# actionml/universal-recommender

Hardware: NVIDIA H100
Metric: CCO train events/sec to indicator model (higher is better)
Workload: dtype int32+f64

## Files before the change

### universal_recommender_b200/csrc/cco_api.cu

```cuda
#include <cuda_runtime.h>
#include <dlfcn.h>
#include <stdarg.h>
#include <stdio.h>
#include <stdlib.h>
#include <string.h>

#include <algorithm>
#include <cmath>
#include <functional>
#include <cub/cub.cuh>
#include <nvtx3/nvToolsExt.h>
#include <condition_variable>
#include <mutex>
#include <string>
#include <thread>
#include <vector>

#include "../../include/cco_b200.h"
#include "cco_kernels.cuh"
#include "cco_sampler.cuh"
#include "cco_format.cuh"
#include "cco_strings.cuh"

namespace cco {
// ... 391 lines not shown
  m.col += m.q_base;
  m.q_base = 0;
  m.nnz = n_unique;
  CK(cudaGetLastError());
  ar.release(flag);
  ar.release(pos);
  ar.release(k0);
  ar.release(k1);
  return CCO_OK;
}

struct HeavyRows {
  int32_t *list = nullptr;
  int *n = nullptr;
};
static int list_heavy_rows(cco_ctx *c, Arena &ar, const DevRaw &raw, HeavyRows *h) {
  CKR(ar.alloc(&h->list, std::max<long long>(raw.n_rows, 1)));
  CKR(ar.alloc(&h->n, 1));
  CK(cudaMemsetAsync(h->n, 0, 4, c->stream));
  if (raw.n_rows > 0) {
    k_list_heavy_rows<<<grid_for(raw.n_rows, 256, c->sm_count), 256, 0, c->stream>>>(raw.n_rows, raw.rp, h->list, h->n);
    c->launches++;
  }
  return CCO_OK;
}
static void launch_check(cco_ctx *c, const DevRaw &raw, const HeavyRows &h, int *flags) {
  if (raw.n_rows <= 0) return;
  const long long q_lo = raw.q_base, q_hi = raw.q_base + raw.nnz;
  k_check_rows<kSG><<<grid_for(raw.n_rows * kSG, 256, c->sm_count), 256, 0, c->stream>>>(raw.n_rows, raw.n_cols, raw.rp, raw.col, q_lo, q_hi,
                                                                                       nullptr, nullptr, flags);
  k_check_rows<32><<<c->sm_count * 4, 256, 0, c->stream>>>(raw.n_rows, raw.n_cols, raw.rp, raw.col, q_lo, q_hi, h.list, h.n, flags);
  c->launches += 2;
}
struct SampleScratch {
  unsigned long long *col_thr = nullptr;
  uint8_t *keep = nullptr;
};
static int sample_scratch(cco_ctx *c, Arena &ar, const DevRaw &raw, const int32_t *raw_counts, int32_t m, SampleScratch *sc) {
  CKR(ar.alloc(&sc->col_thr, std::max<int32_t>(raw.n_cols, 1)));
  CKR(ar.alloc(&sc->keep, std::max<long long>(raw.nnz, 1)));
  if (raw.n_cols > 0) {
    k_col_thresholds<<<grid_for(raw.n_cols, 256, c->sm_count, 4), 256, 0, c->stream>>>(raw.n_cols, raw_counts, m, sc->col_thr);
    c->launches++;
  }
  return CCO_OK;
}
static void launch_count(cco_ctx *c, const DevRaw &raw, const SampleScratch &sc, int32_t m, int32_t seed, uint32_t flags, const int *bad,
                         uint32_t *kept, int32_t *new_counts) {
  if (raw.n_rows <= 0 || raw.nnz <= 0) return;
  const long long q_lo = raw.q_base, q_hi = raw.q_base + raw.nnz;
  const long long n_chunks = (raw.nnz + kSampleChunk - 1) / kSampleChunk;
  k_sample_count<<<grid_for(n_chunks * 32, 256, c->sm_count), 256, 0, c->stream>>>(raw.n_rows, raw.row_base, raw.rp, raw.col, raw.n_cols, q_lo, q_hi,
                                                                                  sc.col_thr, m, seed, flags, bad, kept, new_counts, sc.keep);
  c->launches++;
}
static int launch_write(cco_ctx *c, Arena &ar, const DevRaw &raw, const SampleScratch &sc, int32_t *dst) {
  if (raw.n_rows <= 0 || raw.nnz <= 0) return CCO_OK;
  long long *n_sel;
  CKR(ar.alloc(&n_sel, 1));
  size_t tb = 0;
  CK(cub::DeviceSelect::Flagged(nullptr, tb, raw.col + raw.q_base, sc.keep, dst, n_sel, (long long)raw.nnz, c->stream));
  void *tmp;
  CKR(ar.alloc((char **)&tmp, tb));
  CK(cub::DeviceSelect::Flagged(tmp, tb, raw.col + raw.q_base, sc.keep, dst, n_sel, (long long)raw.nnz, c->stream));
  ar.release(tmp);
  c->launches += 2;
  return CCO_OK;
}

static int downsample_device(cco_ctx *c, Arena &ar, const DevRaw &raw, const int *bad, const int32_t *raw_counts, int32_t m,
                             int32_t seed, uint32_t flags, DevMat *out) {
  out->n_rows = raw.n_rows;
  out->n_cols = raw.n_cols;
  uint32_t *kept;
  CKR(ar.alloc(&kept, raw.n_rows + 1));
  CKR(ar.alloc(&out->rp, raw.n_rows + 1));
  if (!out->marg) CKR(ar.alloc(&out->marg, std::max<int32_t>(raw.n_cols, 1)));
  CKR(ar.alloc(&out->col, std::max<long long>(raw.nnz, 1)));
  CK(cudaMemsetAsync(out->marg, 0, sizeof(int32_t) * std::max<int32_t>(raw.n_cols, 1), c->stream));
  CK(cudaMemsetAsync(kept, 0, sizeof(uint32_t) * ((size_t)raw.n_rows + 1), c->stream));
  SampleScratch sc;
  CKR(sample_scratch(c, ar, raw, raw_counts, m, &sc));
  launch_count(c, raw, sc, m, seed, flags, bad, kept, out->marg);
  CKR(exclusive_sum_u32(c, ar, kept, out->rp, raw.n_rows + 1));
  CKR(launch_write(c, ar, raw, sc, out->col));
  CK(cudaGetLastError());
  ar.release(kept);
  ar.release(sc.col_thr);
  ar.release(sc.keep);
  return CCO_OK;
}

static int nccl_check(int rc, const char *what) {
  if (rc != 0) return set_error(CCO_E_NCCL, "%s: %s", what, g_nccl.GetErrorString(rc));
  return CCO_OK;
}

static int downsample_sharded_all(cco_ctx *c, Arena &ar, const std::vector<DevRaw> &raw, const int *d_check ,
                                  const std::vector<long long> &block_cap,
                                  long long U, const int32_t *raw_counts, int32_t *marg_all, const std::vector<long long> &col_off,
                                  const cco_indicator_params_t *params, int32_t seed, uint32_t flags, std::vector<DevMat> &dm,
                                  cudaEvent_t *stage_ev ) {
  cudaStream_t s = c->stream;
  const int W = c->world, r = c->rank, n_mats = (int)raw.size();
  const long long S = (U + W - 1) / W;
  const long long row_base = raw[0].row_base;
  std::vector<uint32_t *> kept(n_mats, nullptr);
  std::vector<SampleScratch> sc(n_mats);
  for (int i = 0; i < n_mats; ++i) {
    DevMat *out = &dm[i];
    out->n_rows = U;
    out->n_cols = raw[i].n_cols;
    out->marg = marg_all + col_off[i];
    CKR(ar.alloc(&kept[i], (size_t)(W * S + 1)));
    CKR(ar.alloc(&out->rp, U + 1));
    CK(cudaMemsetAsync(kept[i], 0, sizeof(uint32_t) * (size_t)(W * S + 1), s));
    CKR(sample_scratch(c, ar, raw[i], raw_counts + col_off[i], params[i].max_interactions, &sc[i]));
    launch_count(c, raw[i], sc[i], params[i].max_interactions, seed, flags, d_check + 2 * i, kept[i], out->marg);
  }
  CK(cudaEventRecord(stage_ev[0], s));
  if (S > 0) {
    g_nccl.GroupStart();
    for (int i = 0; i < n_mats; ++i) {
      int rc = g_nccl.AllGather(kept[i] + (size_t)r * S, kept[i], (size_t)S, kNcclUint32, c->comm, s);
      if (rc != 0) { g_nccl.GroupEnd(); return nccl_check(rc, "ncclAllGather(kept counts)"); }
    }
    CKR(nccl_check(g_nccl.GroupEnd(), "ncclGroupEnd(kept counts)"));
  }
  if (col_off[n_mats] > 0)
    CKR(nccl_check(g_nccl.AllReduce(marg_all, marg_all, (size_t)col_off[n_mats], kNcclInt32, kNcclSum, c->comm, s), "ncclAllReduce(marginals)"));
  std::vector<int32_t *> gathered(n_mats, nullptr);
  std::vector<uint32_t> edge((size_t)n_mats * (W + 1), 0);
  for (int i = 0; i < n_mats; ++i) {
    CKR(exclusive_sum_u32(c, ar, kept[i], dm[i].rp, U + 1));
    ar.release(kept[i]);
    for (int q = 0; q <= W; ++q) CKR(mail_fetch(c, &edge[(size_t)i * (W + 1) + q], dm[i].rp + std::min<long long>((long long)q * S, U), 4));
  }
  CK(cudaEventRecord(stage_ev[1], s));
  CKR(mail_wait(c));
  std::vector<long long> cap(n_mats, 0);
  for (int i = 0; i < n_mats; ++i) {
    for (int q = 0; q < W; ++q) cap[i] = std::max<long long>(cap[i], (long long)edge[(size_t)i * (W + 1) + q + 1] - edge[(size_t)i * (W + 1) + q]);
    CKR(ar.alloc(&dm[i].col, std::max<long long>(edge[(size_t)i * (W + 1) + W], 1)));
    if (cap[i] == 0) continue;
    CKR(ar.alloc(&gathered[i], (size_t)(cap[i] * W)));
    CKR(launch_write(c, ar, raw[i], sc[i], gathered[i] + (size_t)r * cap[i]));
    ar.release(sc[i].col_thr);
    ar.release(sc[i].keep);
  }
  CK(cudaEventRecord(stage_ev[2], s));
  g_nccl.GroupStart();
// ... 619 lines not shown
  } guard{res};
  std::vector<IndicatorState> ist(n_mats);
  for (auto &x : ist) CKR(pooled_event(c, false, &x.packed));
  cco_stats_t &st = res->stats;
  st.n_mats = n_mats;
  st.n_users = ds->n_users;
  st.ms_h2d = ds->ms_h2d;
  const bool h2d_pending = ds->h2d_pending;
  const long long n_users = ds->n_users;
  std::vector<DevRaw> raw(n_mats);
  for (int i = 0; i < n_mats; ++i) {
    raw[i].n_rows = ds->n_local;
    raw[i].row_base = ds->row_base;
    raw[i].n_cols = (int32_t)ds->n_cols[i];
    raw[i].q_base = ds->q_lo[i];
    raw[i].nnz = ds->q_hi[i] - ds->q_lo[i];
    raw[i].nnz_cap = ds->nnz[i];
    raw[i].rp = ds->rp[i];
    raw[i].col = ds->col[i];
    st.nnz_in_total += ds->nnz[i];
  }
  CK(cudaEventRecord(c->ev[1], s));
  nvtx_push("cco:prepare");
  std::vector<cudaEvent_t> sev(8, nullptr);
  for (auto &e : sev) CKR(pooled_event(c, true, &e));
  auto mark = [&](int k) { return cudaEventRecord(sev[k], s); };
  long long total_cols = 0;
  std::vector<long long> col_off(n_mats + 1, 0);
  for (int i = 0; i < n_mats; ++i) {
    col_off[i] = total_cols;
    total_cols += raw[i].n_cols;
  }
  col_off[n_mats] = total_cols;
  constexpr int kHistCopies = 16;
  const long long copy_stride = std::max<long long>(total_cols, 1);
  int32_t *raw_counts, *marg_all;
  int *d_check;
  CKR(ar.alloc(&raw_counts, (size_t)copy_stride * kHistCopies));
  CKR(ar.alloc(&marg_all, (size_t)copy_stride));
  CKR(ar.alloc(&d_check, 2 * n_mats));
  CK(cudaMemsetAsync(raw_counts, 0, sizeof(int32_t) * (size_t)copy_stride * kHistCopies, s));
  CK(cudaMemsetAsync(marg_all, 0, sizeof(int32_t) * (size_t)copy_stride, s));
  CK(cudaMemsetAsync(d_check, 0, sizeof(int) * 2 * n_mats, s));
  for (int i = 0; i < n_mats; ++i) {
    CK(cudaStreamWaitEvent(s, ds->ready[i], 0));
    if (ds->n_local == 0) continue;
    int *verdict = ds->validated ? nullptr : d_check + 2 * i;
    if (verdict) {
      k_check_row_ptr<<<grid_for(raw[i].n_rows, 256, c->sm_count), 256, 0, s>>>(raw[i].n_rows, raw[i].rp, raw[i].q_base, raw[i].q_base + raw[i].nnz,
                                                                              verdict);
      c->launches++;
    }
    if (raw[i].nnz > 0) {
      k_col_histogram_flat<true><<<grid_for(raw[i].nnz, 256, c->sm_count), 256, 0, s>>>(raw[i].nnz, raw[i].col + raw[i].q_base, raw[i].n_cols,
                                                                                       raw_counts + col_off[i], kHistCopies, copy_stride, verdict);
      c->launches++;
    }
  }
  if (total_cols > 0) {
    k_sum_copies<<<grid_for(total_cols, 256, c->sm_count), 256, 0, s>>>(total_cols, kHistCopies, copy_stride, raw_counts);
    c->launches++;
  }
  CK(mark(0));
  if (c->world > 1) {
    if (total_cols > 0)
      CKR(nccl_check(g_nccl.AllReduce(raw_counts, raw_counts, (size_t)total_cols, kNcclInt32, kNcclSum, c->comm, s), "ncclAllReduce(raw counts)"));
    CKR(nccl_check(g_nccl.AllReduce(d_check, d_check, (size_t)(2 * n_mats), kNcclInt32, kNcclMax, c->comm, s), "ncclAllReduce(check flags)"));
  }
  CK(mark(1));
  std::vector<DevMat> dm(n_mats);
  if (c->world > 1) {
    CKR(downsample_sharded_all(c, ar, raw, d_check, ds->block_cap, n_users, raw_counts, marg_all, col_off, params, seed, flags, dm, &sev[2]));
  } else {
    for (int i = 0; i < n_mats; ++i) {
      dm[i].marg = marg_all + col_off[i];
      CKR(downsample_device(c, ar, raw[i], d_check + 2 * i, raw_counts + col_off[i], params[i].max_interactions, seed, flags, &dm[i]));
    }
    CK(mark(2));
    CK(mark(3));
    CK(mark(4));
    CK(mark(5));
  }
  const int32_t n_items_a = dm[0].n_cols;
  uint32_t *at_ptr, *cursor;
  int32_t *at_users, *d_max;
  CKR(ar.alloc(&at_ptr, n_items_a + 1));
  CKR(ar.alloc(&cursor, n_items_a + 1));
  CKR(ar.alloc(&d_max, n_mats));
  CKR(ar.alloc(&at_users, std::max<long long>(ds->nnz[0], 1)));
  CK(cudaMemsetAsync(d_max, 0, 4 * (size_t)n_mats, s));
  {
    uint32_t *marg_pad;
    CKR(ar.alloc(&marg_pad, n_items_a + 1));
    CK(cudaMemcpyAsync(marg_pad, dm[0].marg, sizeof(int32_t) * (size_t)n_items_a, cudaMemcpyDeviceToDevice, s));
    CK(cudaMemsetAsync(marg_pad + n_items_a, 0, 4, s));
    CKR(exclusive_sum_u32(c, ar, marg_pad, at_ptr, (long long)n_items_a + 1));
    ar.release(marg_pad);
  }
  CK(cudaMemcpyAsync(cursor, at_ptr, sizeof(uint32_t) * ((size_t)n_items_a + 1), cudaMemcpyDeviceToDevice, s));
  k_transpose_scatter<<<grid_for(n_users * kSG, 256, c->sm_count), 256, 0, s>>>(n_users, dm[0].rp, dm[0].col, cursor, at_users);
  c->launches++;
  for (int i = 0; i < n_mats; ++i)
    if (dm[i].n_cols > 0) {
      k_max_i32<<<grid_for(dm[i].n_cols, 256, c->sm_count, 2), 256, 0, s>>>(dm[i].n_cols, dm[i].marg, d_max + i);
      c->launches++;
    }
  std::vector<int32_t> max_marg(n_mats, 0);
  std::vector<uint32_t> h_nnz(n_mats);
  std::vector<int> h_check(2 * n_mats, 0);
  CKR(mail_fetch(c, max_marg.data(), d_max, 4 * (size_t)n_mats));
  CKR(mail_fetch(c, h_check.data(), d_check, sizeof(int) * 2 * (size_t)n_mats));
  for (int i = 0; i < n_mats; ++i) CKR(mail_fetch(c, &h_nnz[i], dm[i].rp + n_users, 4));
  CK(mark(6));
  CK(cudaEventRecord(c->ev[2], s));
  nvtx_pop();
  CKR(mail_wait(c));
  for (int i = 0; i < n_mats; ++i)
    if (h_check[2 * i]) return set_error(CCO_E_INVALID_ARG, "matrix %d: row_ptr not monotone or column index out of [0, n_cols)", i);
  for (int i = 0; i < n_mats && i < 16; ++i) st.nnz_downsampled[i] = h_nnz[i];

  std::vector<IndicatorOut> io(n_mats);
  std::vector<cudaEvent_t> ev_rows(2 * n_mats, nullptr);
  for (auto &e : ev_rows) CKR(pooled_event(c, true, &e));
  for (int i = 0; i < n_mats; ++i) {
    nvtx_push("cco:indicator");
    CKR(enqueue_indicator(c, ar, at_ptr, at_users, n_items_a, dm[0].marg, max_marg[0], max_marg[i], dm[i], n_users, i == 0, params[i],
                          flags, false, c->ev[2], ev_rows[2 * i], ev_rows[2 * i + 1], &ist[i]));
    nvtx_pop();
    if (i > 0) CKR(finish_indicator(c, &ist[i - 1], flags, i - 1, &res->mats[i - 1], &io[i - 1]));
  }
  CKR(finish_indicator(c, &ist[n_mats - 1], flags, n_mats - 1, &res->mats[n_mats - 1], &io[n_mats - 1]));
  CK(cudaEventRecord(c->copy_ev[1], c->copy_stream));
  CK(cudaStreamWaitEvent(s, c->copy_ev[1], 0));
  CK(cudaEventRecord(c->ev[3], s));
// ... 1250 lines not shown
  long long *d[4];
  double *dout;
  const int64_t *h[4] = {k11, k12, k21, k22};
  for (int j = 0; j < 4; ++j) {
    CKR(ar.alloc(&d[j], n));
    CK(cudaMemcpyAsync(d[j], h[j], sizeof(int64_t) * (size_t)n, cudaMemcpyHostToDevice, c->stream));
  }
  CKR(ar.alloc(&dout, n));
  k_debug_llr<<<(unsigned)((n + 255) / 256), 256, 0, c->stream>>>(n, d[0], d[1], d[2], d[3], flags, dout);
  CK(cudaMemcpyAsync(out, dout, sizeof(double) * (size_t)n, cudaMemcpyDeviceToHost, c->stream));
  CK(cudaStreamSynchronize(c->stream));
  CK(cudaGetLastError());
  return CCO_OK;
}

int cco_debug_downsample(cco_ctx_t *c, const cco_csr_t *m, int32_t max_interactions, int32_t seed, uint32_t flags,
                         int64_t **row_ptr, int32_t **col_idx, int32_t *raw_col_counts, int32_t *new_col_counts) {
  if (!c || !m || !row_ptr || !col_idx) return set_error(CCO_E_INVALID_ARG, "null argument");
  if (c->world != 1 || !c->members.empty()) return set_error(CCO_E_UNSUPPORTED, "debug entries need a single-GPU context");
  cco_indicator_params_t prm = {max_interactions, 1, 0, 0.0};
  CKR(validate_host(1, m, &prm));
  CK(cudaSetDevice(c->device));
  mail_reset(c);
  cco_dataset *ds = nullptr;
  CKR(dataset_upload(c, 1, m, flags, &ds));
  struct DG { cco_dataset *d; ~DG() { dataset_release(d); } } dg{ds};
  Arena ar(c->stream);
  DevRaw raw;
  raw.n_rows = ds->n_users; raw.n_cols = (int32_t)ds->n_cols[0]; raw.nnz = ds->nnz[0]; raw.nnz_cap = ds->nnz[0];
  raw.rp = ds->rp[0]; raw.col = ds->col[0];
  int32_t *counts;
  CKR(ar.alloc(&counts, std::max<int32_t>(m->n_cols, 1)));
  CK(cudaMemsetAsync(counts, 0, sizeof(int32_t) * (size_t)std::max<int32_t>(m->n_cols, 1), c->stream));
  if (raw.nnz > 0 && m->n_rows > 0)
    k_col_histogram<<<grid_for(raw.nnz, 256, c->sm_count), 256, 0, c->stream>>>(0, m->n_rows, raw.rp, raw.col, raw.n_cols, counts, 1, 0);
  DevMat dm;
  CKR(downsample_device(c, ar, raw, nullptr, counts, max_interactions, seed, flags, &dm));
  std::vector<uint32_t> rp32((size_t)m->n_rows + 1);
  CK(cudaMemcpyAsync(rp32.data(), dm.rp, sizeof(uint32_t) * rp32.size(), cudaMemcpyDeviceToHost, c->stream));
  if (raw_col_counts && m->n_cols > 0)
    CK(cudaMemcpyAsync(raw_col_counts, counts, sizeof(int32_t) * (size_t)m->n_cols, cudaMemcpyDeviceToHost, c->stream));
  if (new_col_counts && m->n_cols > 0)
    CK(cudaMemcpyAsync(new_col_counts, dm.marg, sizeof(int32_t) * (size_t)m->n_cols, cudaMemcpyDeviceToHost, c->stream));
  CK(cudaStreamSynchronize(c->stream));
  CK(cudaGetLastError());
  size_t nnz = rp32[m->n_rows];
  int64_t *rp = (int64_t *)malloc(sizeof(int64_t) * rp32.size());
  int32_t *ci = (int32_t *)malloc(sizeof(int32_t) * std::max<size_t>(nnz, 1));
  if (!rp || !ci) return set_error(CCO_E_OOM, "malloc failed");
  for (size_t i = 0; i < rp32.size(); ++i) rp[i] = rp32[i];
  if (nnz) CK(cudaMemcpy(ci, dm.col, sizeof(int32_t) * nnz, cudaMemcpyDeviceToHost));
  *row_ptr = rp;
  *col_idx = ci;
  return CCO_OK;
}

int cco_debug_cooccurrence(cco_ctx_t *c, const cco_csr_t *a, const cco_csr_t *b, int64_t **row_ptr, int32_t **col_idx,
                           int32_t **count) {
  if (!c || !a || !b || !row_ptr || !col_idx || !count) return set_error(CCO_E_INVALID_ARG, "null argument");
  if (c->world != 1 || !c->members.empty()) return set_error(CCO_E_UNSUPPORTED, "debug entries need a single-GPU context");
  cco_csr_t two[2] = {*a, *b};
  cco_indicator_params_t prm[2] = {{0x7fffffff, 1, 0, 0.0}, {0x7fffffff, 1, 0, 0.0}};
  CKR(validate_host(2, two, prm));
  CK(cudaSetDevice(c->device));
  mail_reset(c);
  cudaStream_t s = c->stream;
  cco_dataset *ds = nullptr;
  CKR(dataset_upload(c, 2, two, 0, &ds));
  struct DG { cco_dataset *d; ~DG() { dataset_release(d); } } dg{ds};
  Arena ar(s);
  struct CopyJoin {
    cco_ctx *c;
    ~CopyJoin() { cudaStreamSynchronize(c->copy_stream); }
  } copy_join{c};
  std::vector<DevRaw> raw(2);
  for (int i = 0; i < 2; ++i) {
    raw[i].n_rows = ds->n_users; raw[i].n_cols = (int32_t)ds->n_cols[i]; raw[i].nnz = ds->nnz[i]; raw[i].nnz_cap = ds->nnz[i];
    raw[i].rp = ds->rp[i]; raw[i].col = ds->col[i];
  }
  std::vector<DevMat> dm(2);
  for (int i = 0; i < 2; ++i) {
    int32_t *counts;
    CKR(ar.alloc(&counts, std::max<int32_t>(raw[i].n_cols, 1)));
    CK(cudaMemsetAsync(counts, 0, sizeof(int32_t) * (size_t)std::max<int32_t>(raw[i].n_cols, 1), s));
    if (raw[i].nnz > 0 && raw[i].n_rows > 0)
      k_col_histogram<<<grid_for(raw[i].nnz, 256, c->sm_count), 256, 0, s>>>(0, raw[i].n_rows, raw[i].rp, raw[i].col, raw[i].n_cols, counts, 1, 0);
    CKR(downsample_device(c, ar, raw[i], nullptr, counts, 0x7fffffff, 0, 0, &dm[i]));
  }
  const int32_t n_items_a = dm[0].n_cols;
  uint32_t *at_ptr, *cursor, *marg_pad;
  int32_t *at_users, *d_max;
  CKR(ar.alloc(&at_ptr, n_items_a + 1));
  CKR(ar.alloc(&cursor, n_items_a + 1));
  CKR(ar.alloc(&marg_pad, n_items_a + 1));
  CKR(ar.alloc(&d_max, 2));
  CKR(ar.alloc(&at_users, std::max<long long>(raw[0].nnz, 1)));
  CK(cudaMemsetAsync(d_max, 0, 8, s));
  CK(cudaMemcpyAsync(marg_pad, dm[0].marg, sizeof(int32_t) * (size_t)n_items_a, cudaMemcpyDeviceToDevice, s));
  CK(cudaMemsetAsync(marg_pad + n_items_a, 0, 4, s));
  CKR(exclusive_sum_u32(c, ar, marg_pad, at_ptr, (long long)n_items_a + 1));
  CK(cudaMemcpyAsync(cursor, at_ptr, sizeof(uint32_t) * ((size_t)n_items_a + 1), cudaMemcpyDeviceToDevice, s));
  k_transpose_scatter<<<grid_for(a->n_rows * kSG, 256, c->sm_count), 256, 0, s>>>(a->n_rows, dm[0].rp, dm[0].col, cursor, at_users);
  if (n_items_a > 0) k_max_i32<<<grid_for(n_items_a, 256, c->sm_count, 2), 256, 0, s>>>(n_items_a, dm[0].marg, d_max);
  if (dm[1].n_cols > 0) k_max_i32<<<grid_for(dm[1].n_cols, 256, c->sm_count, 2), 256, 0, s>>>(dm[1].n_cols, dm[1].marg, d_max + 1);
  int32_t max_marg_ab[2] = {0, 0};
  CK(cudaMemcpyAsync(max_marg_ab, d_max, 8, cudaMemcpyDeviceToHost, s));
  CK(cudaStreamSynchronize(s));
  CK(cudaGetLastError());
  ResultMat rm;
  IndicatorOut io;
  IndicatorState ist;
  struct EG { IndicatorState &x; ~EG() { if (x.packed) cudaEventDestroy(x.packed); } } eg{ist};
  cco_indicator_params_t p1 = {0x7fffffff, 1, 0, 0.0};
  auto put = [&]() {
    for (void *p : {(void *)rm.row_ptr, (void *)rm.col, (void *)rm.llr, (void *)rm.cnt})
      if (p) c->pinned_put(p);
  };
  int rc = enqueue_indicator(c, ar, at_ptr, at_users, n_items_a, dm[0].marg, max_marg_ab[0], max_marg_ab[1], dm[1], a->n_rows, false, p1,
                             0, true, nullptr, nullptr, nullptr, &ist);
  if (rc == CCO_OK) rc = finish_indicator(c, &ist, 0, 0, &rm, &io);
  cudaStreamSynchronize(c->copy_stream);
  if (rc != CCO_OK) {
    put();
    return rc;
  }
  size_t nnz = (size_t)rm.row_ptr[n_items_a];
  int64_t *rp = (int64_t *)malloc(sizeof(int64_t) * ((size_t)n_items_a + 1));
  int32_t *ci = (int32_t *)malloc(sizeof(int32_t) * std::max<size_t>(nnz, 1));
  int32_t *cn = (int32_t *)malloc(sizeof(int32_t) * std::max<size_t>(nnz, 1));
  if (!rp || !ci || !cn) {
    put();
    return set_error(CCO_E_OOM, "malloc failed");
  }
  memcpy(rp, rm.row_ptr, sizeof(int64_t) * ((size_t)n_items_a + 1));
  std::vector<std::pair<int32_t, int32_t>> tmp;
// ... 19 lines not shown
```

### universal_recommender_b200/csrc/cco_kernels.cuh

```cuda
#pragma once

#include <cuda_runtime.h>
#include <stdint.h>

namespace cco {

struct RowArgs {
  const uint32_t *at_ptr;
  const int32_t *at_users;
  const uint32_t *b_ptr;
  const int32_t *b_col;
  const int32_t *marg_a;
  const int32_t *marg_b;
  const int32_t *key_of_col;
  const int32_t *first_key_of_cb;
  int32_t key_shift;
  const uint2 *ext;
  int32_t max_marg_b;
  const int32_t *rows_sorted;
  const uint32_t *row_work;
  const int32_t *bin_bounds;
  int32_t bin;
  int32_t n_cols_b;
  long long n_users;
// ... 94 lines not shown

constexpr int kHeavyRow = 256;
__global__ void k_list_heavy_rows(long long n_rows, const long long *__restrict__ rp, int32_t *__restrict__ list, int *__restrict__ n_list) {
  for (long long r = blockIdx.x * (long long)blockDim.x + threadIdx.x; r < n_rows; r += (long long)gridDim.x * blockDim.x)
    if (rp[r + 1] - rp[r] > kHeavyRow) list[atomicAdd(n_list, 1)] = (int32_t)r;
}
#define CCO_ROW_LOOP_BEGIN(SG)                                                                         \
  const int lane = threadIdx.x % SG;                                                                   \
  long long it = (blockIdx.x * (long long)blockDim.x + threadIdx.x) / SG;                              \
  const long long stride = (long long)gridDim.x * blockDim.x / SG;                                     \
  const long long n_it = list ? (long long)*n_list : n_rows;                                           \
  for (; it < n_it; it += stride) {                                                                    \
    const long long row = list ? (long long)list[it] : it;
#define CCO_ROW_LOOP_END }

template <int SG>
__global__ void k_check_rows(long long n_rows, int32_t n_cols, const long long *__restrict__ rp, const int32_t *__restrict__ col,
                             long long q_lo, long long q_hi, const int32_t *__restrict__ list, const int *__restrict__ n_list, int *flags) {
  int bad = 0, unsorted = 0;
  CCO_ROW_LOOP_BEGIN(SG)
    long long s = rp[row], e = rp[row + 1];
    if (e < s || s < q_lo || e > q_hi) { bad = 1; continue; }
    if (!list && e - s > kHeavyRow) continue;
    for (long long q = s + lane; q < e; q += SG) {
      int32_t c = col[q];
      if (c < 0 || c >= n_cols) bad = 1;
      if (q > s && col[q - 1] >= c) unsorted = 1;
    }
  CCO_ROW_LOOP_END
  if (bad) atomicOr(&flags[0], 1);
  if (unsorted) atomicOr(&flags[1], 1);
}

__global__ void k_col_histogram(long long row_begin, long long row_end, const long long *__restrict__ rp,
                                const int32_t *__restrict__ col, int32_t n_cols, int32_t *__restrict__ counts, int n_copies,
                                long long copy_stride) {
  const long long s = rp[row_begin], e = rp[row_end];
  const int lane = threadIdx.x & 31;
  int32_t *mine = counts + (long long)(blockIdx.x % n_copies) * copy_stride;
  for (long long q0 = s + blockIdx.x * (long long)blockDim.x + (threadIdx.x & ~31); q0 < e;
       q0 += (long long)gridDim.x * blockDim.x) {
    const long long q = q0 + lane;
    const bool act = q < e;
    const unsigned am = __ballot_sync(0xffffffffu, act);
    if (act) {
      int32_t c = col[q];
      unsigned peers = __match_any_sync(am, c);
      if ((__ffs(peers) - 1) == lane && (uint32_t)c < (uint32_t)n_cols) atomicAdd(&mine[c], __popc(peers));
    }
  }
}
__global__ void k_sum_copies(long long n, int n_copies, long long copy_stride, int32_t *__restrict__ counts) {
  for (long long i = blockIdx.x * (long long)blockDim.x + threadIdx.x; i < n; i += (long long)gridDim.x * blockDim.x) {
    int32_t acc = counts[i];
    for (int k = 1; k < n_copies; ++k) acc += counts[i + k * copy_stride];
    counts[i] = acc;
  }
}

__global__ void k_col_histogram_u32(const uint32_t *__restrict__ lo, const uint32_t *__restrict__ hi,
                                    const int32_t *__restrict__ col, int32_t *__restrict__ counts) {
  const long long s = *lo, e = *hi;
  const int lane = threadIdx.x & 31;
  for (long long q0 = s + blockIdx.x * (long long)blockDim.x + (threadIdx.x & ~31); q0 < e;
       q0 += (long long)gridDim.x * blockDim.x) {
    const long long q = q0 + lane;
    const bool act = q < e;
    const unsigned am = __ballot_sync(0xffffffffu, act);
    if (act) {
      const int32_t c = col[q];
      const unsigned peers = __match_any_sync(am, c);
      if ((__ffs(peers) - 1) == lane) atomicAdd(&counts[c], __popc(peers));
    }
  }
}

__device__ __forceinline__ double row_sample_rate(long long d, int32_t m, bool intdiv) {
  if (d <= 0) return 1.0;
  const long long md = d < m ? d : (long long)m;
  return intdiv ? (double)(md / d) : __ddiv_rn((double)md, (double)d);
}
constexpr unsigned long long kKeepAlways = 1ULL << 53;
__device__ __forceinline__ unsigned long long rate_threshold(double rate) {
  if (rate >= 1.0) return kKeepAlways;
  return (unsigned long long)floor(__dmul_rn(rate, 0x1.0p53));
}
__global__ void k_col_thresholds(int32_t n_cols, const int32_t *__restrict__ raw_counts, int32_t m, unsigned long long *__restrict__ thr) {
  for (int j = blockIdx.x * blockDim.x + threadIdx.x; j < n_cols; j += gridDim.x * blockDim.x) {
    const int32_t c = raw_counts[j];
    thr[j] = c <= m ? kKeepAlways : rate_threshold(__ddiv_rn((double)m, (double)c));
  }
}
// ... 40 lines not shown
                                   long long q_lo, long long q_hi, const uint8_t *__restrict__ keep_flag,
                                   const int32_t *__restrict__ list, const int *__restrict__ n_list,
                                   const uint32_t *__restrict__ new_ptr, const uint32_t *__restrict__ out_base, int32_t *__restrict__ new_col) {
  const int sg_shift = SG == 32 ? 0 : (threadIdx.x & 31) / SG * SG;
  const unsigned sg_mask = SG == 32 ? 0xffffffffu : (((1u << SG) - 1u) << sg_shift);
  const uint32_t base = out_base ? *out_base : 0u;
  CCO_ROW_LOOP_BEGIN(SG)
    long long s = rp[row], e = rp[row + 1], d = e - s;
    if (!list && d > kHeavyRow) continue;
    if (d < 0 || s < q_lo || e > q_hi) continue;
    uint32_t w = new_ptr[row_base + row] - base;
    for (long long q0 = s; q0 < e; q0 += SG) {
      long long q = q0 + lane;
      bool keep = false;
      int32_t j = 0;
      if (q < e) {
        j = col[q];
        keep = keep_flag[q - q_lo] != 0;
      }
      unsigned b = (__ballot_sync(sg_mask, keep) & sg_mask) >> sg_shift;
      if (keep) new_col[w + __popc(b & ((1u << lane) - 1u))] = j;
      w += __popc(b);
    }
  CCO_ROW_LOOP_END
}

__global__ void k_pack_blocks(int world, long long S, long long U, long long cap, const uint32_t *__restrict__ new_ptr,
                              const int32_t *__restrict__ gathered, int32_t *__restrict__ new_col) {
  for (int q = blockIdx.y; q < world; q += gridDim.y) {
    const long long u0 = min((long long)q * S, U), u1 = min(u0 + S, U);
    const uint32_t lo = new_ptr[u0], hi = new_ptr[u1];
    const int32_t *src = gathered + (long long)q * cap;
    for (uint32_t i = blockIdx.x * blockDim.x + threadIdx.x; i < hi - lo; i += gridDim.x * blockDim.x) new_col[lo + i] = src[i];
  }
}

__global__ void k_transpose_scatter(long long n_rows, const uint32_t *__restrict__ rp, const int32_t *__restrict__ col,
                                    uint32_t *__restrict__ cursor, int32_t *__restrict__ users) {
  const int lane = threadIdx.x % kSG;
  long long row = (blockIdx.x * (long long)blockDim.x + threadIdx.x) / kSG;
  const long long stride = (long long)gridDim.x * blockDim.x / kSG;
  for (; row < n_rows; row += stride) {
    uint32_t s = rp[row], e = rp[row + 1];
    for (uint32_t q = s + lane; q < e; q += kSG) users[atomicAdd(&cursor[col[q]], 1u)] = (int32_t)row;
  }
}

__global__ void k_row_work(int32_t n_items, const uint32_t *__restrict__ at_ptr, const int32_t *__restrict__ at_users,
                           const uint32_t *__restrict__ b_ptr, uint32_t *__restrict__ row_work,
                           unsigned long long *__restrict__ work64, int32_t *__restrict__ item_ids,
                           uint2 *__restrict__ ext) {
  const int lane = threadIdx.x % kSG;
  const unsigned sg_mask = ((1u << kSG) - 1u) << ((threadIdx.x & 31) / kSG * kSG);
  int item = (blockIdx.x * blockDim.x + threadIdx.x) / kSG;
  const int stride = gridDim.x * blockDim.x / kSG;
  for (; item < n_items; item += stride) {
    uint32_t s = at_ptr[item], e = at_ptr[item + 1];
    unsigned long long w = 0;
    for (uint32_t q = s + lane; q < e; q += kSG) {
      int32_t u = at_users[q];
      const uint32_t bs = b_ptr[u], bl = b_ptr[u + 1] - bs;
      w += bl;
      if (ext) ext[q] = make_uint2(bs, bl);
    }
#pragma unroll
    for (int o = kSG / 2; o > 0; o >>= 1) w += __shfl_xor_sync(sg_mask, w, o);
    if (lane == 0) {
      row_work[item] = w > 0xffffffffULL ? 0xffffffffu : (uint32_t)w;
      work64[item] = w;
      item_ids[item] = item;
    }
  }
}

struct BinThresholds {
  uint32_t t[12];
};
// ... 782 lines not shown
```

### universal_recommender_b200/csrc/cco_sampler.cuh

```cuda
#pragma once

#include <cuda_runtime.h>
#include <stdint.h>

#include "cco_kernels.cuh"

namespace cco {

constexpr int kSampleChunk = 256;

__device__ __forceinline__ long long warp_find_row(const long long *__restrict__ rp, long long n_rows, long long q, int lane) {
  long long lo = 0, hi = n_rows;
  while (hi - lo > 1) {
    const long long step = (hi - lo + 31) / 32;
    const long long p = lo + lane * step;
    const bool ok = p < hi && rp[p] <= q;
    const unsigned b = __ballot_sync(0xffffffffu, ok) | 1u;
    const int top = 31 - __clz(b);
    lo += top * step;
    hi = hi < lo + step ? hi : lo + step;
  }
  return lo;
}

__global__ void __launch_bounds__(256) k_sample_count(long long n_rows, long long row_base, const long long *__restrict__ rp,
                                                      const int32_t *__restrict__ col, int32_t n_cols, long long q_lo, long long q_hi,
                                                      const unsigned long long *__restrict__ col_thr, int32_t m, int32_t seed, uint32_t flags,
                                                      const int *__restrict__ bad ,
                                                      uint32_t *__restrict__ kept_per_row , int32_t *__restrict__ new_counts,
                                                      uint8_t *__restrict__ keep_flag) {
  const int lane = threadIdx.x & 31;
  const long long warp = (blockIdx.x * (long long)blockDim.x + threadIdx.x) >> 5;
  const long long n_warps = ((long long)gridDim.x * blockDim.x) >> 5;
  const long long n_chunks = (q_hi - q_lo + kSampleChunk - 1) / kSampleChunk;
  const bool intdiv = (flags & CCO_FLAG_ROWRATE_INTDIV) != 0;
  const long long kNoRow = 0x7fffffffffffffffLL;
  if (n_rows <= 0) return;
  if (bad && *bad) {
    for (long long q = blockIdx.x * (long long)blockDim.x + threadIdx.x; q < q_hi - q_lo; q += (long long)gridDim.x * blockDim.x) keep_flag[q] = 0;
    return;
  }
  for (long long chunk = warp; chunk < n_chunks; chunk += n_warps) {
    const long long Q0 = q_lo + chunk * kSampleChunk;
    const long long Q1 = Q0 + kSampleChunk < q_hi ? Q0 + kSampleChunk : q_hi;
    long long base = warp_find_row(rp, n_rows, Q0, lane);
    long long start_i, end_i;
    unsigned long long t_i, x_i;
    uint32_t kept_i;
#define CCO_LOAD_WINDOW()                                                                                   \
  {                                                                                                         \
    const long long r = base + lane;                                                                        \
    start_i = end_i = kNoRow;                                                                               \
    t_i = kKeepAlways;                                                                                      \
    x_i = 0;                                                                                                \
    if (r < n_rows) {                                                                                       \
      start_i = rp[r];                                                                                      \
      end_i = rp[r + 1];                                                                                    \
      const long long d = end_i - start_i;                                                                  \
      if (d > (long long)m) t_i = rate_threshold(row_sample_rate(d, m, intdiv));  \
      x_i = mix64(((uint64_t)(uint32_t)seed << 32) | (uint64_t)(uint32_t)(row_base + r));                   \
    }                                                                                                       \
    kept_i = 0;                                                                                             \
  }
#define CCO_FLUSH_WINDOW()                                                                                  \
  if (kept_i) atomicAdd(&kept_per_row[row_base + base + lane], kept_i);
    CCO_LOAD_WINDOW()
    for (long long qb = Q0; qb < Q1; qb += 32) {
      const long long q = qb + lane;
      bool pending = q < Q1;
      const int32_t j = pending ? col[q] : 0;
      unsigned long long t_col = kKeepAlways;
      if (pending && (uint32_t)j < (uint32_t)n_cols) t_col = col_thr[j];
      while (true) {
        int idx = 0;
#pragma unroll
        for (int step = 16; step > 0; step >>= 1) {
          const long long v = __shfl_sync(0xffffffffu, end_i, idx + step - 1);
          if (v <= q) idx += step;
        }
        {
          const long long v = __shfl_sync(0xffffffffu, end_i, idx);
          if (v <= q) idx += 1;
        }
        const int src = idx & 31;
        const unsigned long long t_row = __shfl_sync(0xffffffffu, t_i, src);
        const unsigned long long x_row = __shfl_sync(0xffffffffu, x_i, src);
        const bool here = pending && idx < 32;
        const bool real_row = base + idx < n_rows;
        bool keep = false;
        if (here) {
          keep = real_row && (uint32_t)j < (uint32_t)n_cols && keep_entry_thr(t_row, t_col, x_row, (uint32_t)j);
          keep_flag[q - q_lo] = keep ? 1 : 0;
          if (keep && new_counts) atomicAdd(&new_counts[j], 1);
        }
        const unsigned kb = __ballot_sync(0xffffffffu, keep);
        const int a = start_i <= qb ? 0 : (start_i >= qb + 32 ? 32 : (int)(start_i - qb));
        const int b = end_i <= qb ? 0 : (end_i >= qb + 32 ? 32 : (int)(end_i - qb));
        if (b > a) {
          const unsigned below_b = b >= 32 ? 0xffffffffu : ((1u << b) - 1u);
          const unsigned below_a = (1u << a) - 1u;
          kept_i += __popc(kb & below_b & ~below_a);
        }
        pending = pending && !here;
        if (!__any_sync(0xffffffffu, pending)) break;
        CCO_FLUSH_WINDOW()
        base += 32;
        if (base >= n_rows) {
          if (pending) keep_flag[q - q_lo] = 0;
          kept_i = 0;
          start_i = end_i = kNoRow;
          break;
        }
        CCO_LOAD_WINDOW()
      }
      if (base >= n_rows) {
        for (long long q2 = qb + 32 + lane; q2 < Q1; q2 += 32) keep_flag[q2 - q_lo] = 0;
        break;
      }
    }
    if (base < n_rows && base + lane < n_rows) { CCO_FLUSH_WINDOW() }
#undef CCO_LOAD_WINDOW
#undef CCO_FLUSH_WINDOW
  }
}

__global__ void k_check_row_ptr(long long n_rows, const long long *__restrict__ rp, long long q_lo, long long q_hi, int *flags) {
  int bad = 0;
  for (long long r = blockIdx.x * (long long)blockDim.x + threadIdx.x; r < n_rows; r += (long long)gridDim.x * blockDim.x) {
    const long long s = rp[r], e = rp[r + 1];
    if (e < s || s < q_lo || e > q_hi) bad = 1;
  }
  if (bad) atomicOr(&flags[0], 1);
}
template <bool AGG>
__global__ void k_col_histogram_flat(long long n, const int32_t *__restrict__ col, int32_t n_cols, int32_t *__restrict__ counts, int n_copies,
                                     long long copy_stride, int *flags ) {
  int32_t *mine = counts + (long long)(blockIdx.x % n_copies) * copy_stride;
  const int lane = threadIdx.x & 31;
  int bad = 0;
  for (long long q0 = blockIdx.x * (long long)blockDim.x + (threadIdx.x & ~31); q0 < n; q0 += (long long)gridDim.x * blockDim.x) {
    const long long q = q0 + lane;
    const bool act = q < n;
    const int32_t j = act ? col[q] : -1;
    const bool ok = act && (uint32_t)j < (uint32_t)n_cols;
    if (act && !ok) bad = 1;
    if (AGG) {
      const unsigned om = __ballot_sync(0xffffffffu, ok);
      if (ok) {
        const unsigned peers = __match_any_sync(om, j);
        if ((__ffs(peers) - 1) == lane) atomicAdd(&mine[j], __popc(peers));
      }
    } else if (ok) {
      atomicAdd(&mine[j], 1);
    }
  }
  if (flags && bad) atomicOr(&flags[0], 1);
}

}
```

Baseline: 4.037 billion.

## Rework column histogram, sampler partitioning, and transpose into entry-balanced kernels

```diff
diff --git a/universal_recommender_b200/csrc/cco_api.cu b/universal_recommender_b200/csrc/cco_api.cu
--- a/universal_recommender_b200/csrc/cco_api.cu
+++ b/universal_recommender_b200/csrc/cco_api.cu
@@ -447,6 +447,22 @@
   k_check_rows<32><<<c->sm_count * 4, 256, 0, c->stream>>>(raw.n_rows, raw.n_cols, raw.rp, raw.col, q_lo, q_hi, h.list, h.n, flags);
   c->launches += 2;
 }
+static int launch_col_histogram(cco_ctx *c, const DevRaw &raw, int32_t *counts, int *verdict, cudaStream_t s) {
+  if (raw.nnz <= 0) return CCO_OK;
+  CK(cudaFuncSetAttribute(k_col_histogram_hot, cudaFuncAttributeMaxDynamicSharedMemorySize, (int)(2 * kHotSlots * sizeof(uint32_t))));
+  const long long grid = std::max<long long>(c->sm_count, (raw.nnz >> 30) + 1);
+  k_col_histogram_hot<<<(unsigned)grid, 1024, 2 * kHotSlots * sizeof(uint32_t), s>>>(raw.nnz, raw.col + raw.q_base, raw.n_cols, counts, verdict);
+  c->launches++;
+  return CCO_OK;
+}
+static int launch_transpose(cco_ctx *c, long long n_rows, const uint32_t *rp, const int32_t *col, uint32_t *cursor, int32_t *users,
+                            cudaStream_t s) {
+  int occ = 1;
+  CK(cudaOccupancyMaxActiveBlocksPerMultiprocessor(&occ, k_transpose_entries, 256, 0));
+  k_transpose_entries<<<c->sm_count * std::max(occ, 1), 256, 0, s>>>(n_rows, rp, col, cursor, users);
+  c->launches++;
+  return CCO_OK;
+}
 struct SampleScratch {
   unsigned long long *col_thr = nullptr;
   uint8_t *keep = nullptr;
@@ -460,14 +476,16 @@
   }
   return CCO_OK;
 }
-static void launch_count(cco_ctx *c, const DevRaw &raw, const SampleScratch &sc, int32_t m, int32_t seed, uint32_t flags, const int *bad,
-                         uint32_t *kept, int32_t *new_counts) {
-  if (raw.n_rows <= 0 || raw.nnz <= 0) return;
+static int launch_count(cco_ctx *c, const DevRaw &raw, const SampleScratch &sc, int32_t m, int32_t seed, uint32_t flags, const int *bad,
+                        uint32_t *kept, int32_t *new_counts) {
+  if (raw.n_rows <= 0 || raw.nnz <= 0) return CCO_OK;
   const long long q_lo = raw.q_base, q_hi = raw.q_base + raw.nnz;
-  const long long n_chunks = (raw.nnz + kSampleChunk - 1) / kSampleChunk;
-  k_sample_count<<<grid_for(n_chunks * 32, 256, c->sm_count), 256, 0, c->stream>>>(raw.n_rows, raw.row_base, raw.rp, raw.col, raw.n_cols, q_lo, q_hi,
+  int occ = 1;
+  CK(cudaOccupancyMaxActiveBlocksPerMultiprocessor(&occ, k_sample_count, 256, 0));
+  k_sample_count<<<grid_for((raw.nnz + 7) / 8, 256, c->sm_count, std::max(occ, 1)), 256, 0, c->stream>>>(raw.n_rows, raw.row_base, raw.rp, raw.col, raw.n_cols, q_lo, q_hi,
                                                                                   sc.col_thr, m, seed, flags, bad, kept, new_counts, sc.keep);
   c->launches++;
+  return CCO_OK;
 }
 static int launch_write(cco_ctx *c, Arena &ar, const DevRaw &raw, const SampleScratch &sc, int32_t *dst) {
   if (raw.n_rows <= 0 || raw.nnz <= 0) return CCO_OK;
@@ -496,7 +514,7 @@
   CK(cudaMemsetAsync(kept, 0, sizeof(uint32_t) * ((size_t)raw.n_rows + 1), c->stream));
   SampleScratch sc;
   CKR(sample_scratch(c, ar, raw, raw_counts, m, &sc));
-  launch_count(c, raw, sc, m, seed, flags, bad, kept, out->marg);
+  CKR(launch_count(c, raw, sc, m, seed, flags, bad, kept, out->marg));
   CKR(exclusive_sum_u32(c, ar, kept, out->rp, raw.n_rows + 1));
   CKR(launch_write(c, ar, raw, sc, out->col));
   CK(cudaGetLastError());
@@ -531,7 +549,7 @@
     CKR(ar.alloc(&out->rp, U + 1));
     CK(cudaMemsetAsync(kept[i], 0, sizeof(uint32_t) * (size_t)(W * S + 1), s));
     CKR(sample_scratch(c, ar, raw[i], raw_counts + col_off[i], params[i].max_interactions, &sc[i]));
-    launch_count(c, raw[i], sc[i], params[i].max_interactions, seed, flags, d_check + 2 * i, kept[i], out->marg);
+    CKR(launch_count(c, raw[i], sc[i], params[i].max_interactions, seed, flags, d_check + 2 * i, kept[i], out->marg));
   }
   CK(cudaEventRecord(stage_ev[0], s));
   if (S > 0) {
@@ -1217,15 +1235,14 @@
     total_cols += raw[i].n_cols;
   }
   col_off[n_mats] = total_cols;
-  constexpr int kHistCopies = 16;
-  const long long copy_stride = std::max<long long>(total_cols, 1);
+  const long long n_counts = std::max<long long>(total_cols, 1);
   int32_t *raw_counts, *marg_all;
   int *d_check;
-  CKR(ar.alloc(&raw_counts, (size_t)copy_stride * kHistCopies));
-  CKR(ar.alloc(&marg_all, (size_t)copy_stride));
+  CKR(ar.alloc(&raw_counts, (size_t)n_counts));
+  CKR(ar.alloc(&marg_all, (size_t)n_counts));
   CKR(ar.alloc(&d_check, 2 * n_mats));
-  CK(cudaMemsetAsync(raw_counts, 0, sizeof(int32_t) * (size_t)copy_stride * kHistCopies, s));
-  CK(cudaMemsetAsync(marg_all, 0, sizeof(int32_t) * (size_t)copy_stride, s));
+  CK(cudaMemsetAsync(raw_counts, 0, sizeof(int32_t) * (size_t)n_counts, s));
+  CK(cudaMemsetAsync(marg_all, 0, sizeof(int32_t) * (size_t)n_counts, s));
   CK(cudaMemsetAsync(d_check, 0, sizeof(int) * 2 * n_mats, s));
   for (int i = 0; i < n_mats; ++i) {
     CK(cudaStreamWaitEvent(s, ds->ready[i], 0));
@@ -1236,15 +1253,7 @@
                                                                               verdict);
       c->launches++;
     }
-    if (raw[i].nnz > 0) {
-      k_col_histogram_flat<true><<<grid_for(raw[i].nnz, 256, c->sm_count), 256, 0, s>>>(raw[i].nnz, raw[i].col + raw[i].q_base, raw[i].n_cols,
-                                                                                       raw_counts + col_off[i], kHistCopies, copy_stride, verdict);
-      c->launches++;
-    }
-  }
-  if (total_cols > 0) {
-    k_sum_copies<<<grid_for(total_cols, 256, c->sm_count), 256, 0, s>>>(total_cols, kHistCopies, copy_stride, raw_counts);
-    c->launches++;
+    CKR(launch_col_histogram(c, raw[i], raw_counts + col_off[i], verdict, s));
   }
   CK(mark(0));
   if (c->world > 1) {
@@ -1283,8 +1292,7 @@
     ar.release(marg_pad);
   }
   CK(cudaMemcpyAsync(cursor, at_ptr, sizeof(uint32_t) * ((size_t)n_items_a + 1), cudaMemcpyDeviceToDevice, s));
-  k_transpose_scatter<<<grid_for(n_users * kSG, 256, c->sm_count), 256, 0, s>>>(n_users, dm[0].rp, dm[0].col, cursor, at_users);
-  c->launches++;
+  CKR(launch_transpose(c, n_users, dm[0].rp, dm[0].col, cursor, at_users, s));
   for (int i = 0; i < n_mats; ++i)
     if (dm[i].n_cols > 0) {
       k_max_i32<<<grid_for(dm[i].n_cols, 256, c->sm_count, 2), 256, 0, s>>>(dm[i].n_cols, dm[i].marg, d_max + i);
@@ -2601,8 +2609,7 @@
   int32_t *counts;
   CKR(ar.alloc(&counts, std::max<int32_t>(m->n_cols, 1)));
   CK(cudaMemsetAsync(counts, 0, sizeof(int32_t) * (size_t)std::max<int32_t>(m->n_cols, 1), c->stream));
-  if (raw.nnz > 0 && m->n_rows > 0)
-    k_col_histogram<<<grid_for(raw.nnz, 256, c->sm_count), 256, 0, c->stream>>>(0, m->n_rows, raw.rp, raw.col, raw.n_cols, counts, 1, 0);
+  if (m->n_rows > 0) CKR(launch_col_histogram(c, raw, counts, nullptr, c->stream));
   DevMat dm;
   CKR(downsample_device(c, ar, raw, nullptr, counts, max_interactions, seed, flags, &dm));
   std::vector<uint32_t> rp32((size_t)m->n_rows + 1);
@@ -2652,8 +2659,7 @@
     int32_t *counts;
     CKR(ar.alloc(&counts, std::max<int32_t>(raw[i].n_cols, 1)));
     CK(cudaMemsetAsync(counts, 0, sizeof(int32_t) * (size_t)std::max<int32_t>(raw[i].n_cols, 1), s));
-    if (raw[i].nnz > 0 && raw[i].n_rows > 0)
-      k_col_histogram<<<grid_for(raw[i].nnz, 256, c->sm_count), 256, 0, s>>>(0, raw[i].n_rows, raw[i].rp, raw[i].col, raw[i].n_cols, counts, 1, 0);
+    if (raw[i].n_rows > 0) CKR(launch_col_histogram(c, raw[i], counts, nullptr, s));
     CKR(downsample_device(c, ar, raw[i], nullptr, counts, 0x7fffffff, 0, 0, &dm[i]));
   }
   const int32_t n_items_a = dm[0].n_cols;
@@ -2669,7 +2675,7 @@
   CK(cudaMemsetAsync(marg_pad + n_items_a, 0, 4, s));
   CKR(exclusive_sum_u32(c, ar, marg_pad, at_ptr, (long long)n_items_a + 1));
   CK(cudaMemcpyAsync(cursor, at_ptr, sizeof(uint32_t) * ((size_t)n_items_a + 1), cudaMemcpyDeviceToDevice, s));
-  k_transpose_scatter<<<grid_for(a->n_rows * kSG, 256, c->sm_count), 256, 0, s>>>(a->n_rows, dm[0].rp, dm[0].col, cursor, at_users);
+  CKR(launch_transpose(c, a->n_rows, dm[0].rp, dm[0].col, cursor, at_users, s));
   if (n_items_a > 0) k_max_i32<<<grid_for(n_items_a, 256, c->sm_count, 2), 256, 0, s>>>(n_items_a, dm[0].marg, d_max);
   if (dm[1].n_cols > 0) k_max_i32<<<grid_for(dm[1].n_cols, 256, c->sm_count, 2), 256, 0, s>>>(dm[1].n_cols, dm[1].marg, d_max + 1);
   int32_t max_marg_ab[2] = {0, 0};
diff --git a/universal_recommender_b200/csrc/cco_kernels.cuh b/universal_recommender_b200/csrc/cco_kernels.cuh
--- a/universal_recommender_b200/csrc/cco_kernels.cuh
+++ b/universal_recommender_b200/csrc/cco_kernels.cuh
@@ -150,32 +150,6 @@
   if (unsorted) atomicOr(&flags[1], 1);
 }
 
-__global__ void k_col_histogram(long long row_begin, long long row_end, const long long *__restrict__ rp,
-                                const int32_t *__restrict__ col, int32_t n_cols, int32_t *__restrict__ counts, int n_copies,
-                                long long copy_stride) {
-  const long long s = rp[row_begin], e = rp[row_end];
-  const int lane = threadIdx.x & 31;
-  int32_t *mine = counts + (long long)(blockIdx.x % n_copies) * copy_stride;
-  for (long long q0 = s + blockIdx.x * (long long)blockDim.x + (threadIdx.x & ~31); q0 < e;
-       q0 += (long long)gridDim.x * blockDim.x) {
-    const long long q = q0 + lane;
-    const bool act = q < e;
-    const unsigned am = __ballot_sync(0xffffffffu, act);
-    if (act) {
-      int32_t c = col[q];
-      unsigned peers = __match_any_sync(am, c);
-      if ((__ffs(peers) - 1) == lane && (uint32_t)c < (uint32_t)n_cols) atomicAdd(&mine[c], __popc(peers));
-    }
-  }
-}
-__global__ void k_sum_copies(long long n, int n_copies, long long copy_stride, int32_t *__restrict__ counts) {
-  for (long long i = blockIdx.x * (long long)blockDim.x + threadIdx.x; i < n; i += (long long)gridDim.x * blockDim.x) {
-    int32_t acc = counts[i];
-    for (int k = 1; k < n_copies; ++k) acc += counts[i + k * copy_stride];
-    counts[i] = acc;
-  }
-}
-
 __global__ void k_col_histogram_u32(const uint32_t *__restrict__ lo, const uint32_t *__restrict__ hi,
                                     const int32_t *__restrict__ col, int32_t *__restrict__ counts) {
   const long long s = *lo, e = *hi;
@@ -282,17 +256,6 @@
     const uint32_t lo = new_ptr[u0], hi = new_ptr[u1];
     const int32_t *src = gathered + (long long)q * cap;
     for (uint32_t i = blockIdx.x * blockDim.x + threadIdx.x; i < hi - lo; i += gridDim.x * blockDim.x) new_col[lo + i] = src[i];
-  }
-}
-
-__global__ void k_transpose_scatter(long long n_rows, const uint32_t *__restrict__ rp, const int32_t *__restrict__ col,
-                                    uint32_t *__restrict__ cursor, int32_t *__restrict__ users) {
-  const int lane = threadIdx.x % kSG;
-  long long row = (blockIdx.x * (long long)blockDim.x + threadIdx.x) / kSG;
-  const long long stride = (long long)gridDim.x * blockDim.x / kSG;
-  for (; row < n_rows; row += stride) {
-    uint32_t s = rp[row], e = rp[row + 1];
-    for (uint32_t q = s + lane; q < e; q += kSG) users[atomicAdd(&cursor[col[q]], 1u)] = (int32_t)row;
   }
 }
 
diff --git a/universal_recommender_b200/csrc/cco_sampler.cuh b/universal_recommender_b200/csrc/cco_sampler.cuh
--- a/universal_recommender_b200/csrc/cco_sampler.cuh
+++ b/universal_recommender_b200/csrc/cco_sampler.cuh
@@ -9,7 +9,8 @@
 
 constexpr int kSampleChunk = 256;
 
-__device__ __forceinline__ long long warp_find_row(const long long *__restrict__ rp, long long n_rows, long long q, int lane) {
+template <typename T>
+__device__ __forceinline__ long long warp_find_row(const T *__restrict__ rp, long long n_rows, long long q, int lane) {
   long long lo = 0, hi = n_rows;
   while (hi - lo > 1) {
     const long long step = (hi - lo + 31) / 32;
@@ -32,21 +33,23 @@
   const int lane = threadIdx.x & 31;
   const long long warp = (blockIdx.x * (long long)blockDim.x + threadIdx.x) >> 5;
   const long long n_warps = ((long long)gridDim.x * blockDim.x) >> 5;
-  const long long n_chunks = (q_hi - q_lo + kSampleChunk - 1) / kSampleChunk;
   const bool intdiv = (flags & CCO_FLAG_ROWRATE_INTDIV) != 0;
-  const long long kNoRow = 0x7fffffffffffffffLL;
+  const uint32_t kNoRow = 0xffffffffu;
   if (n_rows <= 0) return;
   if (bad && *bad) {
     for (long long q = blockIdx.x * (long long)blockDim.x + threadIdx.x; q < q_hi - q_lo; q += (long long)gridDim.x * blockDim.x) keep_flag[q] = 0;
     return;
   }
-  for (long long chunk = warp; chunk < n_chunks; chunk += n_warps) {
-    const long long Q0 = q_lo + chunk * kSampleChunk;
-    const long long Q1 = Q0 + kSampleChunk < q_hi ? Q0 + kSampleChunk : q_hi;
+  {
+    const long long span = ((q_hi - q_lo + n_warps - 1) / n_warps + 31) & ~31LL;
+    const long long Q0 = q_lo + warp * span;
+    if (Q0 >= q_hi) return;
+    const long long Q1 = Q0 + span < q_hi ? Q0 + span : q_hi;
     long long base = warp_find_row(rp, n_rows, Q0, lane);
-    long long start_i, end_i;
+    uint32_t start_i, end_i;
     unsigned long long t_i, x_i;
     uint32_t kept_i;
+    bool win_keep;
 #define CCO_LOAD_WINDOW()                                                                                   \
   {                                                                                                         \
     const long long r = base + lane;                                                                        \
@@ -54,48 +57,55 @@
     t_i = kKeepAlways;                                                                                      \
     x_i = 0;                                                                                                \
     if (r < n_rows) {                                                                                       \
-      start_i = rp[r];                                                                                      \
-      end_i = rp[r + 1];                                                                                    \
-      const long long d = end_i - start_i;                                                                  \
+      const long long s = rp[r], e = rp[r + 1], d = e - s;                                                   \
+      start_i = (uint32_t)(s - q_lo);                                                                       \
+      end_i = (uint32_t)(e - q_lo);                                                                         \
       if (d > (long long)m) t_i = rate_threshold(row_sample_rate(d, m, intdiv));  \
       x_i = mix64(((uint64_t)(uint32_t)seed << 32) | (uint64_t)(uint32_t)(row_base + r));                   \
     }                                                                                                       \
     kept_i = 0;                                                                                             \
+    win_keep = __all_sync(0xffffffffu, t_i == kKeepAlways);                                                 \
   }
 #define CCO_FLUSH_WINDOW()                                                                                  \
   if (kept_i) atomicAdd(&kept_per_row[row_base + base + lane], kept_i);
     CCO_LOAD_WINDOW()
+    const auto thr_of = [&](long long qq, int32_t jj) {
+      return qq < Q1 && (uint32_t)jj < (uint32_t)n_cols ? col_thr[jj] : kKeepAlways;
+    };
+    int32_t j_next = Q0 + lane < Q1 ? col[Q0 + lane] : 0;
+    int32_t j_next2 = Q0 + 32 + lane < Q1 ? col[Q0 + 32 + lane] : 0;
+    unsigned long long t_next = thr_of(Q0 + lane, j_next);
     for (long long qb = Q0; qb < Q1; qb += 32) {
       const long long q = qb + lane;
       bool pending = q < Q1;
-      const int32_t j = pending ? col[q] : 0;
-      unsigned long long t_col = kKeepAlways;
-      if (pending && (uint32_t)j < (uint32_t)n_cols) t_col = col_thr[j];
+      const int32_t j = j_next;
+      const unsigned long long t_col = t_next;
+      t_next = thr_of(q + 32, j_next2);
+      j_next = j_next2;
+      j_next2 = q + 64 < Q1 ? col[q + 64] : 0;
+      const uint32_t qr = (uint32_t)(q - q_lo), qbr = (uint32_t)(qb - q_lo);
       while (true) {
         int idx = 0;
 #pragma unroll
-        for (int step = 16; step > 0; step >>= 1) {
-          const long long v = __shfl_sync(0xffffffffu, end_i, idx + step - 1);
-          if (v <= q) idx += step;
-        }
-        {
-          const long long v = __shfl_sync(0xffffffffu, end_i, idx);
-          if (v <= q) idx += 1;
-        }
+        for (int step = 16; step > 0; step >>= 1)
+          if (__shfl_sync(0xffffffffu, end_i, idx + step - 1) <= qr) idx += step;
+        if (__shfl_sync(0xffffffffu, end_i, idx) <= qr) idx += 1;
         const int src = idx & 31;
-        const unsigned long long t_row = __shfl_sync(0xffffffffu, t_i, src);
-        const unsigned long long x_row = __shfl_sync(0xffffffffu, x_i, src);
+        const unsigned long long t_row = win_keep ? kKeepAlways : __shfl_sync(0xffffffffu, t_i, src);
         const bool here = pending && idx < 32;
         const bool real_row = base + idx < n_rows;
+        const bool live = here && real_row && (uint32_t)j < (uint32_t)n_cols;
+        const bool hashed = live && (t_row < t_col ? t_row : t_col) < kKeepAlways;
+        const unsigned long long x_row = __any_sync(0xffffffffu, hashed) ? __shfl_sync(0xffffffffu, x_i, src) : 0ULL;
         bool keep = false;
         if (here) {
-          keep = real_row && (uint32_t)j < (uint32_t)n_cols && keep_entry_thr(t_row, t_col, x_row, (uint32_t)j);
+          keep = live && keep_entry_thr(t_row, t_col, x_row, (uint32_t)j);
           keep_flag[q - q_lo] = keep ? 1 : 0;
           if (keep && new_counts) atomicAdd(&new_counts[j], 1);
         }
         const unsigned kb = __ballot_sync(0xffffffffu, keep);
-        const int a = start_i <= qb ? 0 : (start_i >= qb + 32 ? 32 : (int)(start_i - qb));
-        const int b = end_i <= qb ? 0 : (end_i >= qb + 32 ? 32 : (int)(end_i - qb));
+        const int a = start_i <= qbr ? 0 : (int)min(start_i - qbr, 32u);
+        const int b = end_i <= qbr ? 0 : (int)min(end_i - qbr, 32u);
         if (b > a) {
           const unsigned below_b = b >= 32 ? 0xffffffffu : ((1u << b) - 1u);
           const unsigned below_a = (1u << a) - 1u;
@@ -132,29 +142,100 @@
   }
   if (bad) atomicOr(&flags[0], 1);
 }
-template <bool AGG>
-__global__ void k_col_histogram_flat(long long n, const int32_t *__restrict__ col, int32_t n_cols, int32_t *__restrict__ counts, int n_copies,
-                                     long long copy_stride, int *flags ) {
-  int32_t *mine = counts + (long long)(blockIdx.x % n_copies) * copy_stride;
+constexpr int kHotSlots = 16384;
+constexpr int kHotProbes = 4;
+constexpr int kHotUnroll = 4;
+constexpr uint32_t kHotFree = 0xffffffffu;
+__global__ void __launch_bounds__(1024) k_col_histogram_hot(long long n, const int32_t *__restrict__ col, int32_t n_cols,
+                                                            int32_t *__restrict__ counts, int *flags ) {
+  extern __shared__ uint32_t hot[];
+  uint32_t *key = hot, *cnt = hot + kHotSlots;
+  for (int i = threadIdx.x; i < kHotSlots; i += blockDim.x) {
+    key[i] = kHotFree;
+    cnt[i] = 0;
+  }
+  __syncthreads();
+  const long long per = (n + gridDim.x - 1) / gridDim.x;
+  const long long lo = min(n, blockIdx.x * per), hi = min(n, lo + per);
+  int bad = 0;
+  for (long long q0 = lo + threadIdx.x; q0 < hi; q0 += (long long)kHotUnroll * blockDim.x) {
+    int32_t j[kHotUnroll];
+#pragma unroll
+    for (int u = 0; u < kHotUnroll; ++u) {
+      const long long q = q0 + (long long)u * blockDim.x;
+      j[u] = q < hi ? col[q] : -1;
+      if (q < hi && (uint32_t)j[u] >= (uint32_t)n_cols) bad = 1;
+    }
+#pragma unroll
+    for (int u = 0; u < kHotUnroll; ++u) {
+      if ((uint32_t)j[u] >= (uint32_t)n_cols) continue;
+      const uint32_t h = ((uint32_t)j[u] * 2654435761u) >> (32 - 14);
+      static_assert(kHotSlots == 1 << 14, "hash width");
+      bool counted = false;
+#pragma unroll
+      for (int p = 0; p < kHotProbes; ++p) {
+        const uint32_t s = (h + p) & (kHotSlots - 1);
+        uint32_t k = ((volatile uint32_t *)key)[s];
+        if (k == kHotFree) k = atomicCAS(&key[s], kHotFree, (uint32_t)j[u]);
+        if (k == kHotFree || k == (uint32_t)j[u]) {
+          atomicAdd(&cnt[s], 1u);
+          counted = true;
+          break;
+        }
+      }
+      if (!counted) atomicAdd(&counts[j[u]], 1);
+    }
+  }
+  __syncthreads();
+  for (int i = threadIdx.x; i < kHotSlots; i += blockDim.x)
+    if (cnt[i]) atomicAdd(&counts[key[i]], (int32_t)cnt[i]);
+  if (flags && bad) atomicOr(&flags[0], 1);
+}
+
+constexpr int kTransposePer = kSampleChunk / 32;
+__global__ void __launch_bounds__(256) k_transpose_entries(long long n_rows, const uint32_t *__restrict__ rp, const int32_t *__restrict__ col,
+                                                           uint32_t *__restrict__ cursor, int32_t *__restrict__ users) {
   const int lane = threadIdx.x & 31;
-  int bad = 0;
-  for (long long q0 = blockIdx.x * (long long)blockDim.x + (threadIdx.x & ~31); q0 < n; q0 += (long long)gridDim.x * blockDim.x) {
-    const long long q = q0 + lane;
-    const bool act = q < n;
-    const int32_t j = act ? col[q] : -1;
-    const bool ok = act && (uint32_t)j < (uint32_t)n_cols;
-    if (act && !ok) bad = 1;
-    if (AGG) {
-      const unsigned om = __ballot_sync(0xffffffffu, ok);
-      if (ok) {
-        const unsigned peers = __match_any_sync(om, j);
-        if ((__ffs(peers) - 1) == lane) atomicAdd(&mine[j], __popc(peers));
-      }
-    } else if (ok) {
-      atomicAdd(&mine[j], 1);
-    }
-  }
-  if (flags && bad) atomicOr(&flags[0], 1);
-}
-
-}
+  const long long warp = (blockIdx.x * (long long)blockDim.x + threadIdx.x) >> 5;
+  const long long n_warps = ((long long)gridDim.x * blockDim.x) >> 5;
+  if (n_rows <= 0) return;
+  const long long nnz = rp[n_rows];
+  const long long span = ((nnz + n_warps - 1) / n_warps + 31) & ~31LL;
+  const long long R0 = warp * span, R1 = R0 + span < nnz ? R0 + span : nnz;
+  if (R0 >= R1) return;
+  long long base = warp_find_row(rp, n_rows, R0, lane);
+  uint32_t end_i = base + lane < n_rows ? rp[base + lane + 1] : 0xffffffffu;
+  for (long long Q0 = R0; Q0 < R1; Q0 += kSampleChunk) {
+    int32_t j[kTransposePer], row[kTransposePer];
+#pragma unroll
+    for (int k = 0; k < kTransposePer; ++k) {
+      const long long q = Q0 + k * 32 + lane;
+      j[k] = q < R1 ? col[q] : -1;
+    }
+#pragma unroll
+    for (int k = 0; k < kTransposePer; ++k) {
+      const uint32_t q = (uint32_t)(Q0 + k * 32 + lane);
+      bool pending = Q0 + k * 32 + lane < R1;
+      row[k] = 0;
+      while (true) {
+        int idx = 0;
+#pragma unroll
+        for (int step = 16; step > 0; step >>= 1)
+          if (__shfl_sync(0xffffffffu, end_i, idx + step - 1) <= q) idx += step;
+        if (__shfl_sync(0xffffffffu, end_i, idx & 31) <= q && idx < 32) idx += 1;
+        if (pending && idx < 32) {
+          row[k] = (int32_t)(base + idx);
+          pending = false;
+        }
+        if (!__any_sync(0xffffffffu, pending)) break;
+        base += 32;
+        end_i = base + lane < n_rows ? rp[base + lane + 1] : 0xffffffffu;
+      }
+    }
+#pragma unroll
+    for (int k = 0; k < kTransposePer; ++k)
+      if (j[k] >= 0) users[atomicAdd(&cursor[j[k]], 1u)] = row[k];
+  }
+}
+
+}
```

Measured after the change: 4.211 billion, median of 6. 1.04x the previous value.
